# cvg/diffmvs

Measured on AMD Instinct MI355X. Metric: depth-maps/sec (640x512, 5 src views), higher is better.
Workload: dtype f32

## Files before the change

diffmvs_amd/_lib.py:

```python
from __future__ import annotations

import ctypes as C
import os

PKG = os.path.dirname(os.path.abspath(__file__))
HIP_LIB_PATH = os.environ.get("DMVS_LIB") or os.path.join(PKG, "libdmvs_hip.so")

ACT_NONE, ACT_RELU, ACT_SIGMOID, ACT_TANH, ACT_SILU = range(5)
IN_PLAIN, IN_UPSAMPLE2, IN_UNSHUFFLE2, IN_ZEROINSERT2 = range(4)
LAYOUT_NCHW, LAYOUT_NHWC, LAYOUT_NHWC_BF16, LAYOUT_NHWC_F16 = 0, 1, 2, 3
DTYPE_F32, DTYPE_BF16, DTYPE_F16, DTYPE_F32_PLAIN = 0, 1, 2, 3
ARITH_F32, ARITH_BF16, ARITH_SPLIT = 0, 1, 2
EW_DEPTH_TO_DISP, EW_DISP_TO_DEPTH = 0, 1

_P = C.c_void_p
_I = C.c_int32
_F = C.c_float


class Conv2dDesc(C.Structure):
    _fields_ = [
        ("in0", _P), ("in1", _P), ("mul0", _P), ("weight", _P), ("scale", _P), ("shift", _P),
        ("residual", _P), ("gru_z", _P), ("gru_h", _P), ("out", _P), ("gn_stats", _P), ("out_mul", _P),
        ("B", _I), ("c0", _I), ("c1", _I), ("Hin", _I), ("Win", _I), ("Hout", _I), ("Wout", _I),
        ("cout", _I), ("cout_pad", _I), ("kh", _I), ("kw", _I), ("stride", _I), ("pad_h", _I), ("pad_w", _I),
        ("in_mode", _I), ("act", _I), ("res_mode", _I), ("res_after_act", _I),
        ("out_layout", _I), ("out_cstride", _I), ("out_coffset", _I), ("gn_groups", _I), ("post_scale", _F),
        ("gate_cstride", _I), ("arith", _I), ("tune", _I), ("out_mul_c0", _I), ("in0_cstride", _I), ("weight_split", _P),
    ]


class Conv3dDesc(C.Structure):
    _fields_ = [
        ("in_", _P), ("weight", _P), ("scale", _P), ("shift", _P), ("residual", _P), ("out", _P),
        ("B", _I), ("cin", _I), ("cout", _I), ("cout_pad", _I),
        ("Din", _I), ("Hin", _I), ("Win", _I), ("Dout", _I), ("Hout", _I), ("Wout", _I),
        ("stride", _I), ("transposed", _I), ("act", _I), ("tune", _I),
    ]


class GetCostDesc(C.Structure):
    _fields_ = [
        ("ref", _P), ("src", _P), ("rt", _P), ("inv_depth", _P), ("confidence", _P), ("view_w", _P),
        ("disp_min", _P), ("disp_max", _P), ("out_cost", _P), ("out_samples", _P), ("worklist", _P),
        ("B", _I), ("S", _I), ("C", _I), ("G", _I), ("n", _I), ("H", _I), ("W", _I), ("vw_shift", _I),
        ("cost_cstride", _I), ("cost_coffset", _I), ("samp_cstride", _I), ("samp_coffset", _I),
        ("interval", _F), ("min_radius", _F), ("max_radius", _F), ("feat_dtype", _I), ("tune", _I),
    ]


SIGNATURES = {
    "dmvs_abi_version": [],
    "dmvs_conv2d_f32": [C.POINTER(Conv2dDesc), _P],
    "dmvs_featurenet_stem_f32": [_P, _P, _P, _P, _P, _P, _P, _P, _I, _I, _I, _I, _P],
    "dmvs_featurenet_stem3_f32": [_P, _P, _P, _P, _P, _P, _P, _P, _P, _P, _P, _I, _I, _I, _I, _P],
    "dmvs_featurenet_conv1_pair_f32": [_P, _P, _P, _P, _P, _P, _P, _P, _I, _I, _I, _I, _P],
    "dmvs_conv2d_wgrad_workspace_f32": [C.POINTER(Conv2dDesc), C.POINTER(C.c_int64)],
    "dmvs_conv2d_wgrad_f32": [C.POINTER(Conv2dDesc), _P, _P, _P, _P, C.c_int64, _P],
    "dmvs_conv3d_f32": [C.POINTER(Conv3dDesc), _P],
    "dmvs_conv3d_wgrad_workspace_f32": [C.POINTER(Conv3dDesc), C.POINTER(C.c_int64)],
    "dmvs_conv3d_wgrad_f32": [C.POINTER(Conv3dDesc), _P, _P, _P, _P, C.c_int64, _P],
    "dmvs_compose_proj_f32": [_P, _P, _I, _I, _P],
    "dmvs_warp_volume_f32": [_P, _P, _P, _P, _I, _I, _I, _I, _I, _I, _I, _P],
    "dmvs_getcost_quad_f32": [C.POINTER(GetCostDesc), _P],
    "dmvs_warp_corr_init_quad_f32": [_P, _P, _P, _P, _P, _P, _I, _I, _I, _I, _I, _I, _I, _I, _I, _I, _I, _P],
    "dmvs_warp_corr_init_bwd_f32": [_P, _P, _P, _P, _P, _P, _P, _P, _I, _I, _I, _I, _I, _I, _I, _I, _I, _I, _P],
    "dmvs_getcost_bwd_f32": [C.POINTER(GetCostDesc), _P, _P, _P, _P],
    "dmvs_view_aggregate_bwd_f32": [_P, _P, _P, _P, _P, _P, _I, _I, _I, _I, _P],
    "dmvs_view_aggregate_f32": [_P, _P, _P, _I, _I, _I, _I, _P],
    "dmvs_sigmoid_max_d_f32": [_P, _P, _I, _I, _I, _P],
    "dmvs_depth_regress_f32": [_P, _P, _P, _P, _P, _P, _I, _I, _I, _P],
    "dmvs_convex_upsample_f32": [_P, _P, _P, _P, _P, _P, _I, _I, _I, _I, _P],
    "dmvs_mask_upsample4_f32": [_P, _P, _P, _F, _P, _P, _P, _P, _P, _I, _I, _I, _I, _I, _P],
    "dmvs_groupnorm_silu_f32": [_P, _P, _P, _P, _P, _P, _P, _I, _I, _I, _I, _F, _P],
    "dmvs_groupnorm_apply_f32": [_P, _P, _P, _P, _P, _P, _P, _I, _I, _I, _I, _F, _P],
    "dmvs_delta_update_f32": [_P, _P, _P, _F, _P, _P, _P, _I, _I, _I, _I, _P],
    "dmvs_depth_convert_f32": [_P, _P, _P, _P, _I, _I, _I, _P],
    "dmvs_act_slice_f32": [_P, _P, _I, _I, _I, _I, _I, _I, _I, _I, _P],
    "dmvs_upsample_nearest_f32": [_P, _P, _I, _I, _I, _I, _P],
    "dmvs_nchw_to_nhwc_f32": [_P, _P, _I, _I, _I, _P],
    "dmvs_groupnorm_silu_bwd_workspace_f32": [_I, _I, _I, C.POINTER(C.c_int64)],
    "dmvs_groupnorm_silu_bwd_f32": [_P, _P, _P, _P, _P, _P, _P, _P, _P, _P, _P, C.c_int64, _I, _I, _I, _I, _F, _P],
    "dmvs_batchnorm_workspace_f32": [_I, _I, _I, _I, C.POINTER(C.c_int64)],
    "dmvs_batchnorm_train_fwd_f32": [_P, _P, _P, _P, _P, _P, _P, _P, _P, C.c_int64, _I, _I, _I, _I, _I, _F, _F, _I, _P],
    "dmvs_batchnorm_train_bwd_f32": [_P, _P, _P, _P, _P, _P, _P, _P, _P, _P, C.c_int64, _I, _I, _I, _I, _I, _I, _P],
    "dmvs_geo_consistency_f32": [_P, _P, _P, _P, _P, _I, _I, _F, _F, _P, _P, _I, _I, _I, _I, _I, _P],
    "dmvs_sumsq_f32": [_P, C.c_int64, _P, _P],
    "dmvs_adamw_step_f32": [_P, _P, _P, _P, C.c_int64, _F, _F, _F, _F, _F, _I, _F, _P, _F, _P],
    "dmvs_view_select_scores_f64": [_P, _P, _P, _P, _P, C.c_int64, C.c_int64, _P, _I, C.c_double, C.c_double, C.c_double, _P, _P, _P],
    "dmvs_cloud_nn_dist_f32": [_P, C.c_int64, _P, C.c_int64, _P, _P, C.c_int64, _P, C.c_double, _P, _F, _P, _P, _P],
    "dmvs_cloud_stats_f32": [_P, _P, C.c_int64, _F, _P, _I, C.c_double, _I, _P, _P],
    "dmvs_cloud_nn_index_f32": [_P, C.c_int64, _P, C.c_int64, _P, _P, C.c_int64, _P, C.c_double, _P, _F, _P, _P, _P, _P, _P],
    "dmvs_cloud_pair_moments_f64": [_P, C.c_int64, _P, _P, C.c_int64, _P, _P, _F, _P, _P, C.c_double, C.c_double, C.c_double, _I, _P, _P],
    "dmvs_cloud_crop_prism_f32": [_P, C.c_int64, _P, _P, _I, _I, C.c_double, C.c_double, _P, _P],
    "dmvs_depth_stats_f32": [_P, _P, _P, C.c_int64, C.c_int64, _P, _I, C.c_double, C.c_double, C.c_double, C.c_double, _I, _P, _P],
    "dmvs_cloud_splat_zmin_f32": [_P, C.c_int64, _P, _P, C.c_int64, _I, _I, C.c_double, C.c_double, C.c_double, _I, _I, _P, _P, _P, _P],
    "dmvs_cloud_splat_sum_f32": [_P, C.c_int64, _P, _P, C.c_int64, _I, _I, C.c_double, C.c_double, C.c_double, C.c_double, C.c_double, _I, _P, _P, _P, _P],
    "dmvs_depth_normals_f32": [_P, _P, _P, C.c_int64, _I, _I, _I, C.c_double, _I, _P, _P, _P],
    "dmvs_tsdf_integrate_f32": [_P, _P, _P, _P, C.c_int64, _I, _I, _I, _I, _I, _P, C.c_double, C.c_double, _I, _P, _P, _P, _P],
    "dmvs_tsdf_flags_u8": [_P, _P, _I, _I, _I, _I, _P, _P, _P],
    "dmvs_tsdf_vertices_f32": [_P, _P, _P, _I, _I, _I, _P, C.c_double, _P, _P, C.c_int64, _P, _P, _P],
    "dmvs_tsdf_faces_i32": [_P, _I, _I, _I, _P, _P, _P, C.c_int64, _P, _P],
}
VIEW_SELECT_MAX_IMAGES, VIEW_SELECT_MAX_LIST = 16384, 1 << 23
CLOUD_MAX_RINGS, CLOUD_MAX_KEY_BITS, CLOUD_MAX_THRESHOLDS = 1024, 62, 16
CLOUD_MOMENTS, CLOUD_MAX_POLYGON = 20, 256
DEPTH_MAX_THRESHOLDS, DEPTH_SLOTS = 8, 7
SPLAT_VIEW_CHUNK, SPLAT_VIEW_DOUBLES, SPLAT_SLOTS, SPLAT_MAX_RADIUS, SPLAT_NO_PRETEST = 8, 15, 4, 16, 0x1
NORMAL_MAX_RADIUS, NORMAL_CAM_DOUBLES, NORMAL_VIEW_CHUNK, NORMAL_SLOTS = 4, 27, 8, 4
TSDF_VIEW_CHUNK, TSDF_VIEW_DOUBLES, TSDF_MAX_VIEWS, TSDF_MAX_QUADS, TSDF_NO_CULL = 8, 12, 65535, 357913941, 0x1
ABI_VERSION = 4
TUNE_NO_WALK, TUNE_PIECES4, TUNE_NO_LEAN, TUNE_1X1_TILED, TUNE_NO_TALL, TUNE_TALL = 0x4, 0x8, 0x100, 0x200, 0x400, 0x800
TUNE3D_PIECES4, TUNE3D_S2_DIRECT, TUNE3D_NO_PAIR = 0x1, 0x2, 0x4
TUNE_SWEEP_GLOBAL = 0x1
TUNE_WGRAD_ACCUMULATE = 0x1000
TUNE_SPLIT_ALL = 0x20000
TUNE_STEM_EXACT = 0x40000


def tune_xcd_group(n: int) -> int:
    return (int(n) & 7) << 14


def tune3d_xcd_group(n: int) -> int:
    return (int(n) & 7) << 4
TUNE_BWD_INTERLEAVED, BWD_GATHER_INTERLEAVED = 0x1, 2


def tune_tile_wx(n: int) -> int:
    return n & 3


def tune_tile_mt(n: int) -> int:
    return (n & 7) << 4


class DmvsError(RuntimeError):
    pass

# ... 32 lines not shown
```

diffmvs_amd/build.py:

```python
from __future__ import annotations

import os
import subprocess
import sys

PKG = os.path.dirname(os.path.abspath(__file__))
ROOT = os.path.dirname(PKG)
CSRC = os.path.join(PKG, "csrc")
LIB = os.path.join(PKG, "libdmvs_hip.so")
PROBE_LIB = os.path.join(PKG, "libdmvs_probe.so")
PROBE_SOURCES = ["probe/getcost_probe.hip", "probe/random_line_gather.hip"]
SOURCES = ["conv2d_k33.hip", "conv2d_k55.hip", "conv2d_k77.hip", "conv2d_k15.hip", "conv2d.hip", "stem.hip", "stem3.hip", "conv1_pair.hip", "conv3d.hip", "warp_quad.hip", "warp_bwd.hip", "warp_bwd_win.hip", "warp_init_bwd_win.hip", "misc.hip", "mask_upsample.hip", "optim.hip", "norm.hip", "fusion.hip", "view_select.hip", "cloud_eval.hip", "cloud_register.hip", "depth_eval.hip", "cloud_render.hip", "depth_normals.hip", "tsdf.hip"]


def _deps():
    out = [os.path.join(ROOT, "include", "dmvs.h"), os.path.join(ROOT, "include", "dmvs_probe.h")]
    for base, _, files in os.walk(CSRC):
        out += [os.path.join(base, f) for f in files]
    return out


def _stale() -> bool:
    if not os.path.exists(LIB) or not os.path.exists(PROBE_LIB):
        return True
    t = min(os.path.getmtime(LIB), os.path.getmtime(PROBE_LIB))
    return any(os.path.getmtime(d) > t for d in _deps())


def build_hip(force: bool = False, save_temps: bool = False, verbose: bool = True) -> str:
    if not force and not _stale():
        return LIB
    import time
    t_start = time.time()
    hipcc = os.environ.get("HIPCC", "/opt/rocm/bin/hipcc")
    flags = ["--offload-arch=gfx950", "-O3", "-std=c++17", "-fPIC",
             "-I", os.path.join(ROOT, "include"), "-I", CSRC,
             "-munsafe-fp-atomics",
             "-Wall", "-Wno-unused-function"]
    objdir = os.path.join(ROOT, "build", "temps" if save_temps else "obj")
    os.makedirs(objdir, exist_ok=True)
    if save_temps:
        flags += ["-save-temps=obj", "-Rpass-analysis=kernel-resource-usage"]

    hdr_t = max(os.path.getmtime(d) for d in _deps() if d.endswith(".h"))

    def compile_one(src):
        obj = os.path.join(objdir, src.replace("/", "_") + ".o")
        if not force and not save_temps and os.path.exists(obj) and os.path.getmtime(obj) > max(hdr_t, os.path.getmtime(os.path.join(CSRC, src))):
            return obj
        cmd = [hipcc] + flags + ["-c", os.path.join(CSRC, src), "-o", obj]
        if verbose:
            print("[diffmvs_amd.build]", " ".join(cmd), flush=True)
        t0 = time.time()
        subprocess.run(cmd, check=True, cwd=objdir if save_temps else ROOT)
        os.utime(obj, (t0, t0))
        return obj

    from concurrent.futures import ThreadPoolExecutor
    with ThreadPoolExecutor(max_workers=min(len(SOURCES), os.cpu_count() or 4)) as pool:
        objs = list(pool.map(compile_one, SOURCES + PROBE_SOURCES))
    for lib, lobjs in ((LIB, objs[:len(SOURCES)]), (PROBE_LIB, objs[len(SOURCES):])):
        link = [hipcc, "--offload-arch=gfx950", "-shared", "-fPIC"] + lobjs + ["-o", lib]
        if verbose:
            print("[diffmvs_amd.build]", " ".join(link), flush=True)
        subprocess.run(link, check=True, cwd=ROOT)
        os.utime(lib, (t_start, t_start))
    return LIB


if __name__ == "__main__":
    build_hip(force="--force" in sys.argv, save_temps="--save-temps" in sys.argv)
    print(LIB)
```

diffmvs_amd/engine.py:

```python
from __future__ import annotations

import math
import os
from typing import Callable, Dict, List, Optional

import torch
import torch.nn.functional as F

from . import ops as K
from .ops import Ops, PackedConv, pack_conv2d, pack_conv3d

_RATIOS = [4, 2, 1]
_MULTS = [(1,), (1, 2), (1, 2, 4)]


def _bn(sd, p):
    return {k: sd[f"{p}.{k}"] for k in ("weight", "bias", "running_mean", "running_var")}


def _cw(sd, p, **kw):
    return pack_conv2d(sd[p + ".conv.weight"], sd.get(p + ".conv.bias"),
                       bn=_bn(sd, p + ".bn") if (p + ".bn.weight") in sd else None, **kw)


def pack_feature(sd, p="feature", g4=False, feat_dtype=torch.float32):
    order = (lambda w: w[K.g4_channels(w.shape[0], feat_dtype).to(w.device)].contiguous()) if g4 else (lambda w: w)
    f = {"conv0.0": _cw(sd, p + ".conv0.0", pad=1), "conv0.1": _cw(sd, p + ".conv0.1", pad=1)}
    for i in (1, 2, 3):
        f[f"conv{i}.0"] = _cw(sd, f"{p}.conv{i}.0", stride=2, pad=2)
        f[f"conv{i}.1"], f[f"conv{i}.2"] = _cw(sd, f"{p}.conv{i}.1", pad=1), _cw(sd, f"{p}.conv{i}.2", pad=1)
    f["out1"] = pack_conv2d(order(sd[p + ".out1.weight"]))
    f["inner1"] = pack_conv2d(sd[p + ".inner1.weight"], sd[p + ".inner1.bias"])
    f["out2"] = pack_conv2d(order(sd[p + ".out2.weight"]), pad=1)
    if (p + ".out3.weight") in sd:
        f["inner2"] = pack_conv2d(sd[p + ".inner2.weight"], sd[p + ".inner2.bias"])
        f["out3"] = pack_conv2d(order(sd[p + ".out3.weight"]), pad=1)
    return f


STEM_FUSE_DEFAULT = "1"


def stem3_applies(o: Ops, x):
    return (o.conv_arith == K.ARITH_SPLIT and os.environ.get("DMVS_STEM_FUSE", STEM_FUSE_DEFAULT) != "0" and
            o.featurenet_stem3_supported(x))


CONV1_PAIR_DEFAULT = "1"


def conv1_pair_applies(o: Ops, c1):
    return (o.conv_arith == K.ARITH_SPLIT and os.environ.get("DMVS_CONV1_PAIR", CONV1_PAIR_DEFAULT) != "0" and
            o.conv1_pair_supported(c1) and c1.shape[3] >= K.Ops.CONV1_PAIR_STRIP)


def run_feature(o: Ops, f, x, layout=K.LAYOUT_NHWC, feat_dtype=torch.float32):
    R = K.ACT_RELU
    if stem3_applies(o, x):
        c1 = o.featurenet_stem3(f["conv0.0"], f["conv0.1"], f["conv1.0"], x)
    else:
        c0 = o.featurenet_stem(f["conv0.0"], f["conv0.1"], x)
        c1 = o.conv2d(f["conv1.0"], c0, act=R)
    if conv1_pair_applies(o, c1):
        c1 = o.conv1_pair(f["conv1.1"], f["conv1.2"], c1)
    else:
        c1 = o.conv2d(f["conv1.2"], o.conv2d(f["conv1.1"], c1, act=R), act=R)
    c2 = o.conv2d(f["conv2.2"], o.conv2d(f["conv2.1"], o.conv2d(f["conv2.0"], c1, act=R), act=R), act=R)
    c3 = o.conv2d(f["conv3.2"], o.conv2d(f["conv3.1"], o.conv2d(f["conv3.0"], c2, act=R), act=R), act=R)
    out = {"stage1": o.conv2d(f["out1"], c3, out_layout=layout, out_dtype=feat_dtype)}
    intra = o.conv2d(f["inner1"], c2, residual=c3, res_mode=K.IN_UPSAMPLE2)
    out["stage2"] = o.conv2d(f["out2"], intra, out_layout=layout, out_dtype=feat_dtype)
    if "out3" in f:
        intra = o.conv2d(f["inner2"], c1, residual=intra, res_mode=K.IN_UPSAMPLE2)
        out["stage3"] = o.conv2d(f["out3"], intra, out_layout=layout, out_dtype=feat_dtype)
    return out


def pack_context_trunk(sd, p="context"):
    c = {"conv1": _cw(sd, p + ".conv1", pad=1)}
    for li in (1, 2, 3):
        for bi in (0, 1):
            q = f"{p}.layer{li}.{bi}"
            c[f"{li}.{bi}.conv1"] = _cw(sd, q + ".conv1", stride=(2 if bi == 0 else 1), pad=1)
            c[f"{li}.{bi}.conv2"] = _cw(sd, q + ".conv2", pad=1)
            if bi == 0:
                c[f"{li}.{bi}.down"] = _cw(sd, q + ".downsample", stride=2, pad=1)
    return c


def run_context_trunk(o: Ops, c, x):
    R = K.ACT_RELU
    x = o.conv2d(c["conv1"], x, act=R)
    taps = {}
    for li in (1, 2, 3):
        y = o.conv2d(c[f"{li}.0.conv1"], x, act=R)
        xd = o.conv2d(c[f"{li}.0.down"], x)
        x = o.conv2d(c[f"{li}.0.conv2"], y, residual=xd, act=R)
        y = o.conv2d(c[f"{li}.1.conv1"], x, act=R)
        x = o.conv2d(c[f"{li}.1.conv2"], y, residual=x, act=R)
        taps[3 - li] = x
    return taps


def pack_pvw(sd, p):
    return (pack_conv3d(sd[p + ".conv.0.conv.weight"], bn=_bn(sd, p + ".conv.0.bn")),
            pack_conv3d(sd[p + ".conv.1.weight"], sd[p + ".conv.1.bias"]))


def run_pvw(o: Ops, pk, cor):
    N, _, D, H, W = cor.shape
    x = o.conv3d(pk[1], o.conv3d(pk[0], cor, act=K.ACT_RELU))
    return o.sigmoid_max_d(x.view(N, D, H, W))


def pack_costreg(sd, p):
    reg = {}
    for i, st in ((0, 1), (1, 1), (2, 2), (3, 1), (4, 2), (5, 1)):
        reg[i] = pack_conv3d(sd[f"{p}.conv{i}.conv.weight"], bn=_bn(sd, f"{p}.conv{i}.bn"), stride=st)
    for i in (6, 7):
        reg[i] = pack_conv3d(sd[f"{p}.conv{i}.conv.weight"], bn=_bn(sd, f"{p}.conv{i}.bn"), stride=2, transposed=True)
    reg["prob"] = pack_conv3d(sd[p + ".prob.weight"])
    return reg


def run_costreg(o: Ops, reg, x):
    R = K.ACT_RELU
    c1 = o.conv3d(reg[1], o.conv3d(reg[0], x, act=R), act=R)
    c3 = o.conv3d(reg[3], o.conv3d(reg[2], c1, act=R), act=R)
    x = o.conv3d(reg[5], o.conv3d(reg[4], c3, act=R), act=R)
    x = o.conv3d(reg[6], x, act=R, residual=c3)
    x = o.conv3d(reg[7], x, act=R, residual=c1)
    return o.conv3d(reg["prob"], x)


def pack_mask(sd, p):
    return (pack_conv2d(sd[p + ".0.weight"], sd[p + ".0.bias"], pad=1), pack_conv2d(sd[p + ".2.weight"], sd[p + ".2.bias"]))


def run_mask(o: Ops, pk, context, post_scale=0.25):
    return o.conv2d(pk[1], o.conv2d(pk[0], context, act=K.ACT_RELU), post_scale=post_scale)


def mask_head_fuses(pk, up_ratio) -> bool:
    return up_ratio == 4 and pk[1].cin == 64 and pk[1].cout == 144 and pk[1].scale is None and os.environ.get("DMVS_MASK_FUSE", "1") != "0"


def pack_gru(sd, p):
    g = {}
    for n, pad in (("1", (0, 2)), ("2", (2, 0))):
        for gate in "zrq":
            g[gate + n] = pack_conv2d(sd[f"{p}.conv{gate}{n}.weight"], sd[f"{p}.conv{gate}{n}.bias"], pad=pad)
        g["zr" + n] = pack_conv2d(torch.cat([sd[f"{p}.convz{n}.weight"], sd[f"{p}.convr{n}.weight"]], 0),
# ... 436 lines not shown
```

diffmvs_amd/ops.py:

```python
from __future__ import annotations

import ctypes as C
import os
from dataclasses import dataclass
from typing import Optional

import torch

from . import _lib
from ._lib import (ACT_NONE, ACT_RELU, ACT_SIGMOID, ACT_SILU, ACT_TANH, ARITH_BF16, ARITH_F32, ARITH_SPLIT, DTYPE_BF16, DTYPE_F16, DTYPE_F32, IN_PLAIN,
                   IN_UNSHUFFLE2, IN_UPSAMPLE2, IN_ZEROINSERT2, LAYOUT_NCHW, LAYOUT_NHWC, LAYOUT_NHWC_BF16, LAYOUT_NHWC_F16)

CONV_ARITH = {"fp32": ARITH_F32, "bf16": ARITH_BF16, "split": ARITH_SPLIT}
FEATURE_DTYPES = {"fp32": torch.float32, "bf16": torch.bfloat16, "fp16": torch.float16}
_DTYPE_CODE = {torch.float32: DTYPE_F32, torch.bfloat16: DTYPE_BF16, torch.float16: DTYPE_F16}
_NHWC_LAYOUT = {torch.float32: LAYOUT_NHWC, torch.bfloat16: LAYOUT_NHWC_BF16, torch.float16: LAYOUT_NHWC_F16}


def _round_up(x: int, m: int) -> int:
    return (x + m - 1) // m * m


@dataclass
class PackedConv:
# ... 266 lines not shown
            kh=kh, kw=kw, stride=pc.stride, pad_h=pc.pad[0], pad_w=pc.pad[1], in_mode=in_mode, act=act,
            res_mode=res_mode, res_after_act=int(res_after_act), out_layout=out_layout, out_cstride=out_cstride,
            out_coffset=out_coffset, post_scale=post_scale, gate_cstride=gate_cstride,
            arith=arith, tune=(self.tune["conv2d"] if tune is None else tune),
            out_mul=_ptr(out_mul), out_mul_c0=out_mul_c0, in0_cstride=in0_cstride)
        self._call("dmvs_conv2d_f32", C.byref(d), self.stream())
        if self.timers is not None and "dmvs_conv2d_f32" in self.timers:
            self.timers.setdefault("_conv2d_flops", []).append(2.0 * B * Hout * Wout * pc.cout * pc.cin * kh * kw)
            self.timers.setdefault("_conv2d_shape", []).append((B, pc.cin, pc.cout, kh, kw, pc.stride, Hout, Wout, in_mode, int(mul0 is not None)))
            nb = sum(t.numel() * t.element_size() for t in (x0, x1, mul0, residual, gru_z, gru_h, out_mul) if t is not None)
            self.timers.setdefault("_conv2d_bytes", []).append(nb + B * Hout * Wout * pc.cout * out.element_size())
        return out

    def featurenet_stem(self, pc0: PackedConv, pc1: PackedConv, x, tune=None):
        if isinstance(x, (list, tuple)):
            self._chk(*x)
            Bv, cin, H, W = x[0].shape
            y = self.empty(len(x) * Bv, 8, H, W)
            for v, xv in enumerate(x):
                self._stem_launch(pc0, pc1, xv, y[v * Bv:(v + 1) * Bv], tune)
            return y
        self._chk(x)
        N, cin, H, W = x.shape
        y = self.empty(N, 8, H, W)
        self._stem_launch(pc0, pc1, x, y, tune)
        return y

    def _stem_launch(self, pc0: PackedConv, pc1: PackedConv, x, y, tune=None):
        N, cin, H, W = x.shape
        if not (cin == 3 and pc0.cin == 3 and pc0.cout == 8 and pc1.cin == 8 and pc1.cout == 8 and pc0.k == (3, 3) and
                pc1.k == (3, 3) and pc0.stride == 1 and pc1.stride == 1 and pc0.pad == (1, 1) and pc1.pad == (1, 1) and
                pc0.cout_pad == 8 and pc1.cout_pad == 8):
            raise _lib.DmvsError("featurenet_stem: expects the 3->8->8 3x3 stem of FeatureNet")
        tune = self.tune["stem"] if tune is None else tune
        if self.conv_arith != ARITH_SPLIT:
            tune |= _lib.TUNE_STEM_EXACT
        self._call("dmvs_featurenet_stem_f32", _ptr(x), _ptr(pc0.weight), _ptr(pc0.scale), _ptr(pc0.shift), _ptr(pc1.weight),
                   _ptr(pc1.scale), _ptr(pc1.shift), _ptr(y), N, H, W, tune, self.stream())

    @staticmethod
    def featurenet_stem3_supported(x):
        xs = x if isinstance(x, (list, tuple)) else [x]
        H, W = xs[0].shape[2], xs[0].shape[3]
        return H % 2 == 0 and W % 4 == 0 and 3 * H * W < 2 ** 31 and all(t.data_ptr() % 16 == 0 for t in xs)

    def featurenet_stem3(self, pc0: PackedConv, pc1: PackedConv, pc2: PackedConv, x, tune=None):
        xs = x if isinstance(x, (list, tuple)) else [x]
        self._chk(*xs)
        Bv, cin, H, W = xs[0].shape
        if not (cin == 3 and pc0.cin == 3 and pc0.cout == 8 and pc1.cin == 8 and pc1.cout == 8 and pc0.k == (3, 3) and
                pc1.k == (3, 3) and pc0.stride == 1 and pc1.stride == 1 and pc0.pad == (1, 1) and pc1.pad == (1, 1) and
                pc0.cout_pad == 8 and pc1.cout_pad == 8 and pc2.cin == 8 and pc2.cout == 16 and pc2.cout_pad == 16 and pc2.k == (5, 5) and
                pc2.stride == 2 and pc2.pad == (2, 2)):
            raise _lib.DmvsError("featurenet_stem3: expects the 3->8->8 3x3 stem of FeatureNet and its 8->16 5x5 stride-2 conv1.0")
        if not self.featurenet_stem3_supported(xs) or any(t.shape != xs[0].shape for t in xs):
            raise _lib.DmvsError(f"featurenet_stem3: needs even H, W % 4 == 0 and 16-byte aligned views of one shape, got {tuple(xs[0].shape)}")
        y = self.empty(len(xs) * Bv, 16, H // 2, W // 2)
        for v, xv in enumerate(xs):
            self._call("dmvs_featurenet_stem3_f32", _ptr(xv), _ptr(pc0.weight), _ptr(pc0.scale), _ptr(pc0.shift), _ptr(pc1.weight),
                       _ptr(pc1.scale), _ptr(pc1.shift), _ptr(pc2.weight), _ptr(pc2.scale), _ptr(pc2.shift), _ptr(y[v * Bv:(v + 1) * Bv]),
                       Bv, H, W, 0 if tune is None else tune, self.stream())
        return y

    CONV1_PAIR_STRIP, CONV1_PAIR_SEGMENT = 80, 64

    @staticmethod
    def conv1_pair_supported(x):
        return (x.dim() == 4 and x.shape[1] == 16 and x.shape[3] % 4 == 0 and 16 * x.shape[2] * x.shape[3] < 2 ** 31 and
                x.data_ptr() % 16 == 0)

    def conv1_pair(self, pc1: PackedConv, pc2: PackedConv, x, tune=0):
        self._chk(x)
        for pc in (pc1, pc2):
            if not (pc.cin == 16 and pc.cout == 16 and pc.cout_pad == 16 and pc.k == (3, 3) and pc.stride == 1 and pc.pad == (1, 1)):
                raise _lib.DmvsError("conv1_pair: expects the two 16->16 3x3 stride-1 layers of FeatureNet's conv1")
        if not self.conv1_pair_supported(x):
            raise _lib.DmvsError(f"conv1_pair: needs 16 channels, W % 4 == 0 and a 16-byte aligned tensor, got {tuple(x.shape)}")
        N, _, H, W = x.shape
        y = self.empty(N, 16, H, W)
        self._call("dmvs_featurenet_conv1_pair_f32", _ptr(x), _ptr(split_weights(pc1)), _ptr(pc1.scale), _ptr(pc1.shift),
                   _ptr(split_weights(pc2)), _ptr(pc2.scale), _ptr(pc2.shift), _ptr(y), N, H, W, tune, self.stream())
        return y

    def conv2d_wgrad(self, pc: PackedConv, x0, grad_out, x1=None, *, mul0=None, in_mode=IN_PLAIN, want_bias=False, tune=None,
                     into_gw=None, into_gb=None):
        self._chk(x0, x1, mul0, grad_out, into_gw, into_gb)
        B = x0.shape[0]
        if in_mode == IN_PLAIN:
            c0, Hin, Win = x0.shape[1], x0.shape[2], x0.shape[3]
        elif in_mode in (IN_UPSAMPLE2, IN_ZEROINSERT2):
            c0, Hin, Win = x0.shape[1], x0.shape[2] * 2, x0.shape[3] * 2
        else:
            c0, Hin, Win = x0.shape[1] * 4, x0.shape[2] // 2, x0.shape[3] // 2
        c1 = 0 if x1 is None else x1.shape[1]
        kh, kw = pc.k
        Hout, Wout = grad_out.shape[2], grad_out.shape[3]
        acc = into_gw is not None
        if acc and (tuple(into_gw.shape) != (pc.cout, pc.cin, kh, kw) or (want_bias and (into_gb is None or tuple(into_gb.shape) != (pc.cout,)))):
            raise _lib.DmvsError("conv2d_wgrad: into_gw / into_gb do not have the gradient's shape")
        gw = into_gw if acc else self.empty(pc.cout, pc.cin, kh, kw)
        gb = (into_gb if acc else self.empty(pc.cout)) if want_bias else None
        d = _lib.Conv2dDesc(
            in0=_ptr(x0), in1=_ptr(x1), mul0=_ptr(mul0), weight=None, scale=None, shift=None, residual=None, gru_z=None,
            gru_h=None, out=None, gn_stats=None, gn_groups=0, B=B, c0=c0, c1=c1, Hin=Hin, Win=Win, Hout=Hout, Wout=Wout,
            cout=pc.cout, cout_pad=pc.cout_pad, kh=kh, kw=kw, stride=pc.stride, pad_h=pc.pad[0], pad_w=pc.pad[1],
            in_mode=in_mode, act=ACT_NONE, res_mode=IN_PLAIN, res_after_act=0, out_layout=LAYOUT_NCHW,
            out_cstride=pc.cout, out_coffset=0, post_scale=1.0, gate_cstride=0, arith=ARITH_F32,
            tune=((self.tune["conv2d"] & _lib.TUNE_PIECES4) if tune is None else tune) | (_lib.TUNE_WGRAD_ACCUMULATE if acc else 0))
        nbytes = C.c_int64(0)
        self._call("dmvs_conv2d_wgrad_workspace_f32", C.byref(d), C.byref(nbytes))
        ws = self.empty(nbytes.value // 4)
        self._call("dmvs_conv2d_wgrad_f32", C.byref(d), _ptr(grad_out), _ptr(gw), _ptr(gb), _ptr(ws), nbytes.value, self.stream())
        if self.timers is not None and "dmvs_conv2d_wgrad_f32" in self.timers:
            self.timers.setdefault("_wgrad_flops", []).append(2.0 * B * Hout * Wout * pc.cout * pc.cin * kh * kw)
        return (gw, gb) if want_bias else gw

    def conv3d(self, pc: PackedConv, x, *, act=ACT_NONE, residual=None, out=None, tune=None):
        self._chk(x, residual, out)
        B, cin, Din, Hin, Win = x.shape
        assert cin == pc.cin
        if pc.transposed:
            Dout, Hout, Wout = 2 * Din, 2 * Hin, 2 * Win
        else:
            s = pc.stride
            Dout, Hout, Wout = (Din - 1) // s + 1, (Hin - 1) // s + 1, (Win - 1) // s + 1
        if out is None:
            out = self.empty(B, pc.cout, Dout, Hout, Wout)
        d = _lib.Conv3dDesc(in_=_ptr(x), weight=_ptr(pc.weight), scale=_ptr(pc.scale), shift=_ptr(pc.shift),
                            residual=_ptr(residual), out=_ptr(out), B=B, cin=cin, cout=pc.cout, cout_pad=pc.cout_pad,
                            Din=Din, Hin=Hin, Win=Win, Dout=Dout, Hout=Hout, Wout=Wout, stride=pc.stride,
                            transposed=int(pc.transposed), act=act, tune=(self.tune["conv3d"] if tune is None else tune))
        self._call("dmvs_conv3d_f32", C.byref(d), self.stream())
        return out

    def conv3d_wgrad(self, x, grad_out, cout, stride, want_bias=False):
        self._chk(x, grad_out)
        B, cin, Din, Hin, Win = x.shape
        Dout, Hout, Wout = grad_out.shape[2:]
        gw = self.empty(cout, cin, 3, 3, 3)
        gb = self.empty(cout) if want_bias else None
        d = _lib.Conv3dDesc(in_=_ptr(x), weight=None, scale=None, shift=None, residual=None, out=None, B=B, cin=cin,
                            cout=cout, cout_pad=_pad_cout(cout), Din=Din, Hin=Hin, Win=Win, Dout=Dout, Hout=Hout, Wout=Wout,
                            stride=stride, transposed=0, act=ACT_NONE)
        nbytes = C.c_int64(0)
        self._call("dmvs_conv3d_wgrad_workspace_f32", C.byref(d), C.byref(nbytes))
        ws = self.empty(nbytes.value // 4)
        self._call("dmvs_conv3d_wgrad_f32", C.byref(d), _ptr(grad_out), _ptr(gw), _ptr(gb), _ptr(ws), nbytes.value, self.stream())
        return (gw, gb) if want_bias else gw

    def compose_proj(self, proj):
        self._chk(proj)
        B, V = proj.shape[0], proj.shape[1]
        out = self.empty(B, V - 1, 12)
        self._call("dmvs_compose_proj_f32", _ptr(proj), _ptr(out), B, V, self.stream())
        return out

    def warp_corr_init_quad(self, ref, src, rt, disp_min, disp_max, D, G=4, tune=None, plain=False):
        self._chk(rt, disp_min, disp_max)
        fdt = self._chk_feat(ref, src)
        if plain and fdt == DTYPE_F32:
            fdt = _lib.DTYPE_F32_PLAIN
        B, H, W, Cc = ref.shape
        S, _, Hs, Ws, _ = src.shape
        out = self.empty(B, S, G, D, H, W)
        self._call("dmvs_warp_corr_init_quad_f32", _ptr(ref), _ptr(src), _ptr(rt), _ptr(disp_min), _ptr(disp_max), _ptr(out),
                   B, S, Cc, G, D, H, W, Hs, Ws, fdt, self.tune["sweep"] if tune is None else tune, self.stream())
# ... 521 lines not shown
```

include/dmvs.h:

```cpp
#ifndef DMVS_H
#define DMVS_H

#include <stdint.h>

#ifdef __cplusplus
extern "C" {
#endif

#define DMVS_ABI_VERSION 4
#define DMVS_EINVAL (-22)

enum { DMVS_ACT_NONE = 0, DMVS_ACT_RELU = 1, DMVS_ACT_SIGMOID = 2, DMVS_ACT_TANH = 3, DMVS_ACT_SILU = 4 };
enum { DMVS_IN_PLAIN = 0, DMVS_IN_UPSAMPLE2 = 1 , DMVS_IN_UNSHUFFLE2 = 2 ,
       DMVS_IN_ZEROINSERT2 = 3  };
enum { DMVS_LAYOUT_NCHW = 0, DMVS_LAYOUT_NHWC = 1,
       DMVS_LAYOUT_NHWC_BF16 = 2, DMVS_LAYOUT_NHWC_F16 = 3 };
enum { DMVS_DTYPE_F32 = 0 , DMVS_DTYPE_BF16 = 1, DMVS_DTYPE_F16 = 2 ,
       DMVS_DTYPE_F32_PLAIN = 3  };

int dmvs_abi_version(void);

#define DMVS_ARITH_F32 0
#define DMVS_ARITH_BF16 1
#define DMVS_ARITH_SPLIT 2

#define DMVS_TUNE_TILE_WX(n) ((n) & 3)
#define DMVS_TUNE_NO_WALK 0x4
#define DMVS_TUNE_PIECES4 0x8
#define DMVS_TUNE_TILE_MT(n) (((n) & 7) << 4)
#define DMVS_TUNE_1X1_TILED 0x200
#define DMVS_TUNE_NO_LEAN 0x100
#define DMVS_TUNE_TALL(n) (((n) & 3) << 10)
#define DMVS_TUNE_STEM_EXACT 0x40000
#define DMVS_TUNE_SPLIT_ALL 0x20000
#define DMVS_TUNE_XCD_GROUP(n) (((n) & 7) << 14)

typedef struct dmvs_conv2d_desc {
    const float* in0;
    const float* in1;
    const float* mul0;
    const float* weight;
    const float* scale;
    const float* shift;
    const float* residual;
    const float* gru_z;
    const float* gru_h;
    float* out;
    double* gn_stats;
    const float* out_mul;
    int32_t B, c0, c1;
    int32_t Hin, Win;
    int32_t Hout, Wout;
    int32_t cout, cout_pad;
    int32_t kh, kw, stride, pad_h, pad_w;
    int32_t in_mode, act;
    int32_t res_mode;
    int32_t res_after_act;
    int32_t out_layout, out_cstride, out_coffset;
    int32_t gn_groups;
    float post_scale;
    int32_t gate_cstride;
    int32_t arith;
    int32_t tune;
    int32_t out_mul_c0;
    int32_t in0_cstride;
    const void* weight_split;
} dmvs_conv2d_desc;

int dmvs_conv2d_f32(const dmvs_conv2d_desc* d, void* stream);

int dmvs_featurenet_stem_f32(const float* x, const float* w0, const float* scale0, const float* shift0, const float* w1,
                             const float* scale1, const float* shift1, float* y, int32_t N, int32_t H, int32_t W, int32_t tune,
                             void* stream);

int dmvs_featurenet_stem3_f32(const float* x, const float* w0, const float* scale0, const float* shift0, const float* w1,
                              const float* scale1, const float* shift1, const float* w2, const float* scale2, const float* shift2,
                              float* y, int32_t N, int32_t H, int32_t W, int32_t tune, void* stream);

int dmvs_featurenet_conv1_pair_f32(const float* x, const void* wsplit1, const float* scale1, const float* shift1, const void* wsplit2,
                                   const float* scale2, const float* shift2, float* y, int32_t N, int32_t H, int32_t W, int32_t tune,
                                   void* stream);

#define DMVS_TUNE_WGRAD_ACCUMULATE 0x1000
int dmvs_conv2d_wgrad_workspace_f32(const dmvs_conv2d_desc* d, int64_t* bytes);
int dmvs_conv2d_wgrad_f32(const dmvs_conv2d_desc* d, const float* grad_out, float* gw, float* gb, float* workspace,
                          int64_t workspace_bytes, void* stream);

typedef struct dmvs_conv3d_desc {
    const float* in;
    const float* weight;
    const float* scale;
    const float* shift;
    const float* residual;
    float* out;
    int32_t B, cin, cout, cout_pad;
    int32_t Din, Hin, Win;
    int32_t Dout, Hout, Wout;
    int32_t stride;
    int32_t transposed;
    int32_t act;
    int32_t tune;
} dmvs_conv3d_desc;
#define DMVS_TUNE3D_PIECES4 0x1
#define DMVS_TUNE3D_S2_DIRECT 0x2
#define DMVS_TUNE3D_NO_PAIR 0x4
#define DMVS_TUNE3D_XCD_GROUP(n) (((n) & 7) << 4)

int dmvs_conv3d_f32(const dmvs_conv3d_desc* d, void* stream);

int dmvs_conv3d_wgrad_workspace_f32(const dmvs_conv3d_desc* d, int64_t* bytes);
int dmvs_conv3d_wgrad_f32(const dmvs_conv3d_desc* d, const float* grad_out, float* gw, float* gb, float* workspace,
                          int64_t workspace_bytes, void* stream);

int dmvs_compose_proj_f32(const float* proj, float* out, int32_t B, int32_t V, void* stream);

#define DMVS_GETCOST_TILE 16
#define DMVS_GETCOST_MAX_WINDOW_VIEWS 16
#define DMVS_GETCOST_WORKLIST_INTS(B, H, W) \
    (4 + 66 * (B) * (((H) + DMVS_GETCOST_TILE - 1) / DMVS_GETCOST_TILE) * (((W) + DMVS_GETCOST_TILE - 1) / DMVS_GETCOST_TILE))
typedef struct dmvs_getcost_desc {
    const float* ref;
    const float* src;
    const float* rt;
    const float* inv_depth;
    const float* confidence;
    const float* view_w;
    const float* disp_min;
    const float* disp_max;
    float* out_cost;
    float* out_samples;
    int32_t* worklist;
    int32_t B, S, C, G, n, H, W;
    int32_t vw_shift;
    int32_t cost_cstride, cost_coffset, samp_cstride, samp_coffset;
    float interval, min_radius, max_radius;
    int32_t feat_dtype;
    int32_t tune;
} dmvs_getcost_desc;

#define DMVS_TUNE_SWEEP_GLOBAL 0x1
int dmvs_getcost_quad_f32(const dmvs_getcost_desc* d, void* stream);
int dmvs_warp_corr_init_quad_f32(const void* ref, const void* src, const float* rt,
                                 const float* disp_min, const float* disp_max, float* out,
                                 int32_t B, int32_t S, int32_t C, int32_t G, int32_t D,
                                 int32_t H, int32_t W, int32_t Hs, int32_t Ws, int32_t feat_dtype, int32_t tune, void* stream);

int dmvs_warp_volume_f32(const float* src, const float* rt, const float* depth, float* out,
                         int32_t B, int32_t C, int32_t D, int32_t H, int32_t W, int32_t Hs, int32_t Ws,
                         void* stream);

#define DMVS_TUNE_BWD_INTERLEAVED 0x1
#define DMVS_BWD_GATHER_INTERLEAVED 2
int dmvs_warp_corr_init_bwd_f32(const float* ref, const float* src, const float* rt,
                                const float* disp_min, const float* disp_max, const float* gcor,
                                float* gref, float* gsrc, int32_t B, int32_t S, int32_t C, int32_t G,
                                int32_t D, int32_t H, int32_t W, int32_t Hs, int32_t Ws, int32_t gather, void* stream);
int dmvs_getcost_bwd_f32(const dmvs_getcost_desc* d, const float* gcost, float* gref, float* gsrc, void* stream);
int dmvs_view_aggregate_bwd_f32(const float* cor, const float* w, const float* out, const float* gout,
                                float* gcor, float* gw, int32_t B, int32_t S, int32_t GD, int32_t HW,
                                void* stream);

int dmvs_view_aggregate_f32(const float* cor, const float* w, float* out,
                            int32_t B, int32_t S, int32_t GD, int32_t HW, void* stream);

int dmvs_sigmoid_max_d_f32(const float* x, float* out, int32_t N, int32_t D, int32_t HW, void* stream);
// ... 136 lines not shown
```

Before: 1514.

## Fuse FPN inner 1x1 conv, upsampled residual and 3x3 output conv

```diff
diff --git a/diffmvs_amd/_lib.py b/diffmvs_amd/_lib.py
--- a/diffmvs_amd/_lib.py
+++ b/diffmvs_amd/_lib.py
@@ -55,6 +55,7 @@
     "dmvs_featurenet_stem_f32": [_P, _P, _P, _P, _P, _P, _P, _P, _I, _I, _I, _I, _P],
     "dmvs_featurenet_stem3_f32": [_P, _P, _P, _P, _P, _P, _P, _P, _P, _P, _P, _I, _I, _I, _I, _P],
     "dmvs_featurenet_conv1_pair_f32": [_P, _P, _P, _P, _P, _P, _P, _P, _I, _I, _I, _I, _P],
+    "dmvs_featurenet_fpn_tail_f32": [_P, _P, _P, _P, _P, _P, _I, _I, _I, _I, _P],
     "dmvs_conv2d_wgrad_workspace_f32": [C.POINTER(Conv2dDesc), C.POINTER(C.c_int64)],
     "dmvs_conv2d_wgrad_f32": [C.POINTER(Conv2dDesc), _P, _P, _P, _P, C.c_int64, _P],
     "dmvs_conv3d_f32": [C.POINTER(Conv3dDesc), _P],
diff --git a/diffmvs_amd/build.py b/diffmvs_amd/build.py
--- a/diffmvs_amd/build.py
+++ b/diffmvs_amd/build.py
@@ -10,7 +10,7 @@
 LIB = os.path.join(PKG, "libdmvs_hip.so")
 PROBE_LIB = os.path.join(PKG, "libdmvs_probe.so")
 PROBE_SOURCES = ["probe/getcost_probe.hip", "probe/random_line_gather.hip"]
-SOURCES = ["conv2d_k33.hip", "conv2d_k55.hip", "conv2d_k77.hip", "conv2d_k15.hip", "conv2d.hip", "stem.hip", "stem3.hip", "conv1_pair.hip", "conv3d.hip", "warp_quad.hip", "warp_bwd.hip", "warp_bwd_win.hip", "warp_init_bwd_win.hip", "misc.hip", "mask_upsample.hip", "optim.hip", "norm.hip", "fusion.hip", "view_select.hip", "cloud_eval.hip", "cloud_register.hip", "depth_eval.hip", "cloud_render.hip", "depth_normals.hip", "tsdf.hip"]
+SOURCES = ["conv2d_k33.hip", "conv2d_k55.hip", "conv2d_k77.hip", "conv2d_k15.hip", "conv2d.hip", "stem.hip", "stem3.hip", "conv1_pair.hip", "fpn_tail.hip", "conv3d.hip", "warp_quad.hip", "warp_bwd.hip", "warp_bwd_win.hip", "warp_init_bwd_win.hip", "misc.hip", "mask_upsample.hip", "optim.hip", "norm.hip", "fusion.hip", "view_select.hip", "cloud_eval.hip", "cloud_register.hip", "depth_eval.hip", "cloud_render.hip", "depth_normals.hip", "tsdf.hip"]
 
 
 def _deps():
diff --git a/diffmvs_amd/csrc/fpn_tail.hip b/diffmvs_amd/csrc/fpn_tail.hip
--- /dev/null
+++ b/diffmvs_amd/csrc/fpn_tail.hip
@@ -0,0 +1,262 @@
+
+#include "dmvs_common.h"
+#include "dmvs_bf16.h"
+#include "dmvs_lds_poison.h"
+
+namespace {
+
+typedef float f32x4 __attribute__((ext_vector_type(4)));
+typedef uint32_t u32x4s __attribute__((ext_vector_type(4)));
+typedef uint32_t u32x2s __attribute__((ext_vector_type(2)));
+
+constexpr int PB = 256;
+constexpr int US = 32, UR = 64;
+constexpr int NP = US + 2;
+constexpr int SLOTS = 4, NCH = 8;
+constexpr int PLQ = SLOTS * NCH * NP;
+constexpr int RINGQ = 3 * PLQ;
+constexpr int SW = US + 8;
+constexpr int C2PIECE = 2 * 32 * SW / 4;
+constexpr int CW = US / 2 + 8;
+constexpr int C3PIECE = 64 * CW / 4;
+constexpr int LDSF = RINGQ * 4 + C2PIECE * 4 + 2 * C3PIECE * 4;
+constexpr int NSTEP = NCH * 3;
+
+__device__ __attribute__((aligned(16))) const float fpn_tail_zero16[4] = {0.0f, 0.0f, 0.0f, 0.0f};
+#define DMVS_LDS_P(p) ((__attribute__((address_space(3))) void*)(p))
+#ifdef DMVS_HOST_EMULATION
+#define DMVS_OPAQUE(v) ((void)0)
+#else
+#define DMVS_OPAQUE(v) asm volatile("" : "+v"(v))
+#endif
+
+__global__ void __launch_bounds__(PB) __attribute__((amdgpu_waves_per_eu(2, 2)))
+featurenet_fpn_tail_kernel(const float* __restrict__ c2, const float* __restrict__ c3, const float* __restrict__ w1, const float* __restrict__ b1,
+                           const u32x4s* __restrict__ ws2, float* __restrict__ y, int N, int H, int W, int nsx, int nsy) {
+    __shared__ __attribute__((aligned(16))) float lds[LDSF];
+    DMVS_LDS_POISON(lds);
+
+    const int tid = threadIdx.x, lane = tid & 63, wave = __builtin_amdgcn_readfirstlane(tid >> 6);
+    const int m = lane & 15, kq = lane >> 4;
+    const int H2 = H >> 1, W2 = W >> 1;
+    const int iplane = H * W, iplane3 = H2 * W2;
+    const int nunits = nsx * nsy * N;
+
+    float w1r[8], b1r[4];
+#pragma unroll
+    for (int c = 0; c < 8; ++c) w1r[c] = w1[(4 * c + kq) * 64 + 16 * wave + m];
+#pragma unroll
+    for (int r = 0; r < 4; ++r) b1r[r] = b1 ? b1[16 * wave + 4 * kq + r] : 0.0f;
+    const int nt = wave & 1, rr = wave >> 1;
+    unsigned lwb = (unsigned)(kq * 32 + nt * 16 + m) * 16u;
+    auto wload = [&](int sp) -> u32x4s {
+        return *reinterpret_cast<const u32x4s*>(reinterpret_cast<const char*>(ws2 + sp * 128) + lwb);
+    };
+    int taps = 0;
+#pragma unroll
+    for (int g = 0; g < 3; ++g) {
+        const int t = min(4 * g + kq, 8);
+        taps |= ((t / 3) | ((t % 3) << 2)) << (4 * g);
+    }
+    u32x4s* const ring = reinterpret_cast<u32x4s*>(lds);
+    float* const st2 = lds + RINGQ * 4;
+    float* const st3 = st2 + C2PIECE * 4;
+
+    int lm = m, ltid = tid;
+
+    for (int unit = blockIdx.x; unit < nunits; unit += gridDim.x) {
+        const int sx = unit % nsx;
+        const int uq = unit / nsx;
+        const int sy = uq % nsy, n = uq / nsy;
+        const int X0 = US * sx, Y0 = UR * sy;
+        const int Yend = min(Y0 + UR, H) - 1;
+        const int Q = (Yend - Y0 + 1) >> 1;
+        const float* const c2b = c2 + (long)n * 32 * iplane;
+        const float* const c3b = c3 + (long)n * 64 * iplane3;
+        float* const yb = y + (long)n * 32 * iplane;
+
+        auto stage_c3 = [&](int row3, int lt) {
+#pragma unroll
+            for (int k = 0; k < 2; ++k) {
+                if (k * PB + wave * 64 < C3PIECE) {
+                    const int e = k * PB + lt;
+                    const int ch = e / (CW / 4), pc = e - ch * (CW / 4);
+                    const int col = (X0 >> 1) - 4 + 4 * pc;
+                    const bool ok = row3 >= 0 && row3 < H2 && col >= 0 && col < W2;
+                    const float* srcp = ok ? c3b + (ch * iplane3 + row3 * W2 + col) : fpn_tail_zero16;
+                    float* dstp = st3 + (((row3 + 2) & 1) * C3PIECE + k * PB + wave * 64) * 4;
+                    __builtin_amdgcn_global_load_lds(srcp, DMVS_LDS_P(dstp), 16, 0, 0);
+                }
+            }
+        };
+        auto stage = [&](int p, bool with_above, int lt) {
+#pragma unroll
+            for (int k = 0; k < 3; ++k) {
+                if (k * PB + wave * 64 < C2PIECE) {
+                    const int e = k * PB + lt;
+                    const int li = e / (C2PIECE / 2), rem = e - li * (C2PIECE / 2);
+                    const int ch = rem / (SW / 4), pc = rem - ch * (SW / 4);
+                    const int row = Y0 - 1 + 2 * p + li, col = X0 - 4 + 4 * pc;
+                    const bool ok = row >= 0 && row < H && col >= 0 && col < W;
+                    const float* srcp = ok ? c2b + (ch * iplane + row * W + col) : fpn_tail_zero16;
+                    float* dstp = st2 + (k * PB + wave * 64) * 4;
+                    __builtin_amdgcn_global_load_lds(srcp, DMVS_LDS_P(dstp), 16, 0, 0);
+                }
+            }
+            stage_c3((Y0 >> 1) + p, lt);
+            if (with_above) stage_c3((Y0 >> 1) + p - 1, lt);
+        };
+        stage(0, true, ltid);
+        DMVS_DMA_BARRIER();
+
+        for (int j = 0; j < Q + 2; ++j) {
+            DMVS_OPAQUE(lm);
+            DMVS_OPAQUE(ltid);
+            DMVS_OPAQUE(lwb);
+            const bool do_out = j >= 2, do_in = j <= Q;
+            const int orow = Y0 + 2 * (j - 2) + rr;
+            f32x4 oacc[2] = {{0.0f, 0.0f, 0.0f, 0.0f}, {0.0f, 0.0f, 0.0f, 0.0f}};
+            if (do_out) {
+                auto qp_of = [&](int s) {
+                    const int c = s / 3, g = s - c * 3;
+                    const int tg = taps >> (4 * g);
+                    const int slot = (orow + 3 + (tg & 3)) & 3;
+                    return (slot * NCH + c) * NP + lm + ((tg >> 2) & 3);
+                };
+                u32x4s wq[3][3];
+                bf16x8 pq[2][2][3];
+#pragma unroll
+                for (int s0 = 0; s0 < 2; ++s0)
+#pragma unroll
+                    for (int pl = 0; pl < 3; ++pl) wq[s0][pl] = wload(s0 * 3 + pl);
+                {
+                    const int qp = qp_of(0);
+#pragma unroll
+                    for (int grp = 0; grp < 2; ++grp)
+#pragma unroll
+                        for (int pl = 0; pl < 3; ++pl) pq[0][grp][pl] = __builtin_bit_cast(bf16x8, ring[pl * PLQ + qp + 16 * grp]);
+                }
+#pragma unroll
+                for (int s = 0; s < NSTEP; ++s) {
+                    const int wb = s % 3, pb = s & 1;
+                    __builtin_amdgcn_sched_barrier(0);
+                    if (s + 2 < NSTEP) {
+#pragma unroll
+                        for (int pl = 0; pl < 3; ++pl) wq[(s + 2) % 3][pl] = wload((s + 2) * 3 + pl);
+                    }
+                    if (s + 1 < NSTEP) {
+                        const int qn = qp_of(s + 1);
+#pragma unroll
+                        for (int grp = 0; grp < 2; ++grp)
+#pragma unroll
+                            for (int pl = 0; pl < 3; ++pl) pq[pb ^ 1][grp][pl] = __builtin_bit_cast(bf16x8, ring[pl * PLQ + qn + 16 * grp]);
+                    }
+                    __builtin_amdgcn_sched_barrier(0);
+                    const bf16x8 wh = __builtin_bit_cast(bf16x8, wq[wb][0]), wm = __builtin_bit_cast(bf16x8, wq[wb][1]),
+                                 wlo = __builtin_bit_cast(bf16x8, wq[wb][2]);
+#pragma unroll
+                    for (int grp = 0; grp < 2; ++grp) oacc[grp] = dmvs_mfma_bf16(wh, pq[pb][grp][2], oacc[grp]);
+#pragma unroll
+                    for (int grp = 0; grp < 2; ++grp) oacc[grp] = dmvs_mfma_bf16(wlo, pq[pb][grp][0], oacc[grp]);
+#pragma unroll
+                    for (int grp = 0; grp < 2; ++grp) oacc[grp] = dmvs_mfma_bf16(wm, pq[pb][grp][1], oacc[grp]);
+#pragma unroll
+                    for (int grp = 0; grp < 2; ++grp) oacc[grp] = dmvs_mfma_bf16(wh, pq[pb][grp][1], oacc[grp]);
+#pragma unroll
+                    for (int grp = 0; grp < 2; ++grp) oacc[grp] = dmvs_mfma_bf16(wm, pq[pb][grp][0], oacc[grp]);
+#pragma unroll
+                    for (int grp = 0; grp < 2; ++grp) oacc[grp] = dmvs_mfma_bf16(wh, pq[pb][grp][0], oacc[grp]);
+                }
+                __builtin_amdgcn_sched_barrier(0);
+            }
+            float iv[6][4];
+            if (do_in) {
+#pragma unroll
+                for (int it = 0; it < 6; ++it) {
+                    const int li = it / 3, grp = it - li * 3;
+                    const int row = Y0 - 1 + 2 * j + li;
+                    const int pp = min(grp * 16 + lm, NP - 1);
+                    const float* xp = st2 + (li * 32 + kq) * SW + 3 + pp;
+                    f32x4 a = {0.0f, 0.0f, 0.0f, 0.0f};
+#pragma unroll
+                    for (int c = 0; c < 8; ++c) a = __builtin_amdgcn_mfma_f32_16x16x4f32(w1r[c], xp[4 * c * SW], a, 0, 0, 0);
+                    const int col = X0 - 1 + pp;
+                    const bool inside = row >= 0 && row < H && col >= 0 && col < W;
+                    const float* rp = st3 + ((((row + 4) >> 1) & 1) * 64 + 16 * wave + 4 * kq) * CW + ((pp - 1) >> 1) + 4;
+#pragma unroll
+                    for (int r = 0; r < 4; ++r) {
+                        const float v = (a[r] + b1r[r]) + rp[r * CW];
+                        iv[it][r] = inside ? v : 0.0f;
+                    }
+                }
+            }
+            DMVS_LDS_BARRIER();
+            if (j + 1 <= Q) stage(j + 1, false, ltid);
+            if (do_out) {
+#pragma unroll
+                for (int grp = 0; grp < 2; ++grp) {
+                    const int col = X0 + grp * 16 + m;
+                    if (col < W) *reinterpret_cast<f32x4*>(yb + ((orow * W + col) * 32 + nt * 16 + 4 * kq)) = oacc[grp];
+                }
+            }
+            if (do_in) {
+#pragma unroll
+                for (int it = 0; it < 6; ++it) {
+                    const int li = it / 3, grp = it - li * 3;
+                    const int row = Y0 - 1 + 2 * j + li;
+                    const int pp = grp * 16 + m;
+                    if (pp < NP) {
+                        float v[8];
+#pragma unroll
+                        for (int r = 0; r < 4; ++r) {
+                            v[r] = iv[it][r];
+                            v[4 + r] = 0.0f;
+                        }
+                        bf16x8 h8, m8, l8;
+                        dmvs_split3_bf16x8(v, h8, m8, l8);
+                        u32x2s* const d = reinterpret_cast<u32x2s*>(ring + ((((row + 4) & 3) * NCH + 2 * wave + (kq >> 1)) * NP + pp)) + (kq & 1);
+                        auto pack4 = [](const bf16x8& b) {
+                            return u32x2s{(uint32_t)(uint16_t)b[0] | ((uint32_t)(uint16_t)b[1] << 16), (uint32_t)(uint16_t)b[2] | ((uint32_t)(uint16_t)b[3] << 16)};
+                        };
+                        d[0] = pack4(h8);
+                        d[PLQ * 2] = pack4(m8);
+                        d[2 * PLQ * 2] = pack4(l8);
+                    }
+                }
+            }
+            DMVS_DMA_BARRIER();
+        }
+    }
+}
+
+#ifdef DMVS_HOST_EMULATION
+int fpn_tail_resident() { return 2; }
+#else
+int fpn_tail_resident() {
+    int dev = 0, per_cu = 0;
+    hipDeviceProp_t prop;
+    if (hipGetDevice(&dev) != hipSuccess || hipGetDeviceProperties(&prop, dev) != hipSuccess) return 512;
+    if (hipOccupancyMaxActiveBlocksPerMultiprocessor(&per_cu, reinterpret_cast<const void*>(featurenet_fpn_tail_kernel), PB, 0) != hipSuccess || per_cu < 1)
+        per_cu = 1;
+    return per_cu * prop.multiProcessorCount;
+}
+#endif
+
+}
+
+extern "C" int dmvs_featurenet_fpn_tail_f32(const float* c2, const float* c3, const float* w_inner, const float* b_inner, const void* wsplit_out,
+                                            float* y, int32_t N, int32_t H, int32_t W, int32_t tune, void* stream) {
+    if (!c2 || !c3 || !w_inner || !wsplit_out || !y || N <= 0 || H <= 0 || W <= 0) return DMVS_EINVAL;
+    if ((H & 1) || (W & 7) || (long)64 * H * W >= (1L << 31)) return DMVS_EINVAL;
+    if ((((uintptr_t)c2 | (uintptr_t)c3 | (uintptr_t)y | (uintptr_t)wsplit_out) & 15) || ((uintptr_t)w_inner & 3) || ((uintptr_t)b_inner & 3))
+        return DMVS_EINVAL;
+    const int nsx = (W + US - 1) / US, nsy = (H + UR - 1) / UR;
+    const long nunits = (long)nsx * nsy * N;
+    if (nunits >= (1L << 31)) return DMVS_EINVAL;
+    static const int resident = fpn_tail_resident();
+    long grid = (tune & 0xffff) ? (tune & 0xffff) : resident;
+    if (grid > nunits) grid = nunits;
+    hipLaunchKernelGGL(featurenet_fpn_tail_kernel, dim3((unsigned)grid), dim3(PB), 0, (hipStream_t)stream, c2, c3, w_inner, b_inner,
+                       reinterpret_cast<const u32x4s*>(wsplit_out), y, N, H, W, nsx, nsy);
+    return dmvs_launch_status();
+}
diff --git a/diffmvs_amd/engine.py b/diffmvs_amd/engine.py
--- a/diffmvs_amd/engine.py
+++ b/diffmvs_amd/engine.py
@@ -52,6 +52,14 @@
 def conv1_pair_applies(o: Ops, c1):
     return (o.conv_arith == K.ARITH_SPLIT and os.environ.get("DMVS_CONV1_PAIR", CONV1_PAIR_DEFAULT) != "0" and
             o.conv1_pair_supported(c1) and c1.shape[3] >= K.Ops.CONV1_PAIR_STRIP)
+
+
+FPN_TAIL_DEFAULT = "1"
+
+
+def fpn_tail_applies(o: Ops, f, c2, c3, layout, feat_dtype):
+    return (o.conv_arith == K.ARITH_SPLIT and layout == K.LAYOUT_NHWC and feat_dtype == torch.float32 and "out3" not in f and
+            os.environ.get("DMVS_FPN_TAIL", FPN_TAIL_DEFAULT) != "0" and o.fpn_tail_supported(c2, c3))
 
 
 def run_feature(o: Ops, f, x, layout=K.LAYOUT_NHWC, feat_dtype=torch.float32):
@@ -68,6 +76,9 @@
     c2 = o.conv2d(f["conv2.2"], o.conv2d(f["conv2.1"], o.conv2d(f["conv2.0"], c1, act=R), act=R), act=R)
     c3 = o.conv2d(f["conv3.2"], o.conv2d(f["conv3.1"], o.conv2d(f["conv3.0"], c2, act=R), act=R), act=R)
     out = {"stage1": o.conv2d(f["out1"], c3, out_layout=layout, out_dtype=feat_dtype)}
+    if fpn_tail_applies(o, f, c2, c3, layout, feat_dtype):
+        out["stage2"] = o.fpn_tail(f["inner1"], f["out2"], c2, c3)
+        return out
     intra = o.conv2d(f["inner1"], c2, residual=c3, res_mode=K.IN_UPSAMPLE2)
     out["stage2"] = o.conv2d(f["out2"], intra, out_layout=layout, out_dtype=feat_dtype)
     if "out3" in f:
diff --git a/diffmvs_amd/ops.py b/diffmvs_amd/ops.py
--- a/diffmvs_amd/ops.py
+++ b/diffmvs_amd/ops.py
@@ -372,6 +372,31 @@
                    _ptr(split_weights(pc2)), _ptr(pc2.scale), _ptr(pc2.shift), _ptr(y), N, H, W, tune, self.stream())
         return y
 
+    FPN_TAIL_STRIP, FPN_TAIL_SEGMENT = 32, 64
+
+    @staticmethod
+    def fpn_tail_supported(c2, c3):
+        if not (c2.dim() == 4 and c3.dim() == 4 and c2.dtype == torch.float32 and c3.dtype == torch.float32):
+            return False
+        N, C, H, W = c2.shape
+        return (C == 32 and H % 2 == 0 and W % 8 == 0 and H > 0 and W > 0 and tuple(c3.shape) == (N, 64, H // 2, W // 2) and
+                64 * H * W < 2 ** 31 and c2.is_contiguous() and c3.is_contiguous() and c2.data_ptr() % 16 == 0 and c3.data_ptr() % 16 == 0)
+
+    def fpn_tail(self, pc_inner: PackedConv, pc_out: PackedConv, c2, c3, tune=0):
+        self._chk(c2, c3)
+        if not (pc_inner.cin == 32 and pc_inner.cout == 64 and pc_inner.cout_pad == 64 and pc_inner.k == (1, 1) and pc_inner.stride == 1 and
+                pc_inner.pad == (0, 0) and pc_inner.scale is None and pc_out.cin == 64 and pc_out.cout == 32 and pc_out.cout_pad == 32 and
+                pc_out.k == (3, 3) and pc_out.stride == 1 and pc_out.pad == (1, 1) and pc_out.scale is None and pc_out.shift is None):
+            raise _lib.DmvsError("fpn_tail: expects FeatureNet's inner1 (32->64 1x1, bias) and out2 (64->32 3x3, no bias)")
+        if not self.fpn_tail_supported(c2, c3):
+            raise _lib.DmvsError(f"fpn_tail: needs c2 [N,32,H,W] and c3 [N,64,H/2,W/2] with even H, W % 8 == 0, contiguous and 16-byte aligned, "
+                                 f"got {tuple(c2.shape)} and {tuple(c3.shape)}")
+        N, _, H, W = c2.shape
+        y = self.empty(N, H, W, 32)
+        self._call("dmvs_featurenet_fpn_tail_f32", _ptr(c2), _ptr(c3), _ptr(pc_inner.weight), _ptr(pc_inner.shift), _ptr(split_weights(pc_out)),
+                   _ptr(y), N, H, W, tune, self.stream())
+        return y
+
     def conv2d_wgrad(self, pc: PackedConv, x0, grad_out, x1=None, *, mul0=None, in_mode=IN_PLAIN, want_bias=False, tune=None,
                      into_gw=None, into_gb=None):
         self._chk(x0, x1, mul0, grad_out, into_gw, into_gb)
diff --git a/include/dmvs.h b/include/dmvs.h
--- a/include/dmvs.h
+++ b/include/dmvs.h
@@ -81,6 +81,9 @@
                                    const float* scale2, const float* shift2, float* y, int32_t N, int32_t H, int32_t W, int32_t tune,
                                    void* stream);
 
+int dmvs_featurenet_fpn_tail_f32(const float* c2, const float* c3, const float* w_inner, const float* b_inner, const void* wsplit_out,
+                                 float* y, int32_t N, int32_t H, int32_t W, int32_t tune, void* stream);
+
 #define DMVS_TUNE_WGRAD_ACCUMULATE 0x1000
 int dmvs_conv2d_wgrad_workspace_f32(const dmvs_conv2d_desc* d, int64_t* bytes);
 int dmvs_conv2d_wgrad_f32(const dmvs_conv2d_desc* d, const float* grad_out, float* gw, float* gb, float* workspace,
```

After: 1530, median of 6. 1.0% higher.
